# blacksnail789521/IMM-TSF

Measured on AMD Instinct MI355X. Metric: forecast windows/sec (train fwd+bwd) on ragged 64-entity batch, higher is better.
Workload: dtype bf16

## Files before the change

imm-tsf_amd/csrc/capi.hip:

```cpp
#include "../../include/immtsf.h"
#include "attn.hpp"
#include "gemm.hpp"
#include "rowops.hpp"
#include "seam_small.hpp"
#include "tail.hpp"
#include "block_util.hpp"
#include <atomic>

namespace { std::atomic<int> g_side_enabled{0}; }

extern "C" {

int immtsf_side_stream_enabled(void) { return g_side_enabled; }
int immtsf_set_side_stream(int32_t on) { g_side_enabled.store(on ? 1 : 0); return 0; }

int immtsf_gemm(int32_t layout, int32_t precision, const float* A, int32_t lda, const float* B, int32_t ldb, float* C,
                int32_t ldc, const float* bias, int32_t M, int32_t N, int32_t K, float alpha, int32_t accumulate,
                int32_t act, immtsf_stream_t stream) {
    if (!A || !B || !C || layout < 0 || layout > 2) return IMMTSF_EINVAL;
    GemmArgs g = gemm_args(M, N, K, lda, ldb, ldc);
    set_problem(g, 0, A, B, C, bias);
    g.alpha = alpha;
    g.accumulate = accumulate;
    g.act = act;
// ... 126 lines not shown

int immtsf_softmax_rows_backward(float* dA, const float* P, int32_t B, int32_t H, int32_t L, int32_t S, float p_drop,
                                 uint64_t seed, uint64_t site, const uint64_t* seed_step_dev, immtsf_stream_t stream) {
    if (!dA || !P) return IMMTSF_EINVAL;
    DropCfg d = mk_drop(p_drop, seed);
    d.seed_dev = seed_step_dev;
    return launch_softmax_rows_bwd(dA, P, B, H, L, S, d, site, static_cast<hipStream_t>(stream));
}

int immtsf_attention_short_forward(const float* qkv, int32_t B, int32_t L, int32_t H, int32_t E, float scale, int32_t causal,
                                   float p_drop, uint64_t seed, uint64_t site, const uint64_t* seed_step_dev, float* out,
                                   immtsf_stream_t stream) {
    if (!qkv || !out || B < 0 || L <= 0 || H <= 0 || E <= 0) return IMMTSF_EINVAL;
    DropCfg d = mk_drop(p_drop, seed);
    d.seed_dev = seed_step_dev;
    return launch_attn_short_fwd(qkv, B, L, H, E, scale, causal, d, site, out, static_cast<hipStream_t>(stream));
}

int immtsf_attention_short_backward(const float* qkv, const float* dout, int32_t B, int32_t L, int32_t H, int32_t E, float scale,
                                    int32_t causal, float p_drop, uint64_t seed, uint64_t site, const uint64_t* seed_step_dev,
                                    float* dqkv, immtsf_stream_t stream) {
    if (!qkv || !dout || !dqkv || B < 0 || L <= 0 || H <= 0 || E <= 0) return IMMTSF_EINVAL;
    DropCfg d = mk_drop(p_drop, seed);
    d.seed_dev = seed_step_dev;
    return launch_attn_short_bwd(qkv, dout, B, L, H, E, scale, causal, d, site, dqkv, static_cast<hipStream_t>(stream));
}

int immtsf_seam_route(int32_t rows, int32_t d, int32_t PW) { return seam_p_fwd_shape_ok(rows, d, PW) ? 1 : 0; }

int immtsf_seam_p_bf16(const void* A, const void* W, const float* bias, float* P, int32_t rows, int32_t d, int32_t PW, immtsf_stream_t stream) {
    return launch_seam_p_fwd(A, W, bias, P, rows, d, PW, static_cast<hipStream_t>(stream));
}

int immtsf_layernorm_backward_lowrank(const float* G, int32_t ldg, int32_t PW, const float* basis, int32_t rows, int32_t d, const float* gamma,
                                      const float* xhat, const void* xhat_h, const float* rstd, float* dx, void* dxh, float p_drop,
                                      const void* keep, int32_t keep_T, const uint8_t* row_flag, int32_t flag_div, float* dgamma, float* dbeta,
                                      float* dxsum, float* scratch, size_t scratch_bytes, int32_t form, immtsf_stream_t stream) {
    if (scratch_bytes < (size_t)256 * 3 * d * sizeof(float) || (form != 0 && form != 1)) return IMMTSF_EINVAL;
    if (p_drop > 0.f && !keep) return IMMTSF_EINVAL;
    return launch_layernorm_bwd_lr(G, ldg, PW, basis, rows, d, gamma, xhat, xhat_h, rstd, dx, dxh, mk_drop(p_drop, 0), 0, dgamma, dbeta, dxsum,
                                   scratch, row_flag, flag_div, static_cast<hipStream_t>(stream), keep, keep_T, form);
}

int immtsf_layernorm_forward(const float* x, int32_t rows, int32_t d, const float* gamma, const float* beta, float eps,
                             float* xhat, float* rstd, float* z, float p_drop, uint64_t seed, uint64_t site,
                             immtsf_stream_t stream) {
    if (!x || !gamma || !beta || !z || d <= 0) return IMMTSF_EINVAL;
    return launch_layernorm_fwd(x, rows, d, gamma, beta, eps, xhat, rstd, z, mk_drop(p_drop, seed), site,
                                static_cast<hipStream_t>(stream));
}

int immtsf_layernorm_backward(float* dz_dy, int32_t rows, int32_t d, const float* gamma, const float* xhat,
                              const float* rstd, float* dx, float* dgamma, float* dbeta, float* scratch, float p_drop,
                              uint64_t seed, uint64_t site, immtsf_stream_t stream) {
    if (!dz_dy || !gamma || !xhat || !rstd || !dx || d <= 0) return IMMTSF_EINVAL;
    hipStream_t s = static_cast<hipStream_t>(stream);
    CHECK(launch_layernorm_bwd(dz_dy, rows, d, gamma, xhat, rstd, dx, mk_drop(p_drop, seed), site, s));
    if (dgamma && dbeta) {
        if (!scratch) return IMMTSF_EINVAL;
        return launch_colsum2(dz_dy, xhat, rows, d, d, dgamma, dbeta, scratch, s);
    }
    if (dgamma) {
        if (!scratch) return IMMTSF_EINVAL;
        CHECK(launch_colsum(dz_dy, xhat, rows, nullptr, d, d, dgamma, 0, scratch, s));
    }
    if (dbeta) {
// ... 172 lines not shown
```

imm-tsf_amd/csrc/seam_small.hip:

```cpp
#include "seam_small.hpp"

namespace {

template <int NT>
__global__ __launch_bounds__(256) void seam_p_fwd_kernel(const bf16_t* __restrict__ A, const bf16_t* __restrict__ W, const float* __restrict__ bias,
                                                          float* __restrict__ out, int rows, int d, int PW) {
    __shared__ f32x4 red[3][NT][64];
    const int tid = threadIdx.x, lane = tid & 63, wave = tid >> 6, fr = lane & 15, fq = lane >> 4;
    const int row = blockIdx.x * 16 + fr;
    const bool rok = row < rows;
    const bf16_t* ap = A + (size_t)(rok ? row : 0) * d + fq * 8;
    const bf16_t* wp[NT];
    bool wok[NT];
#pragma unroll
    for (int j = 0; j < NT; ++j) {
        wok[j] = j * 16 + fr < PW;
        wp[j] = W + (size_t)(wok[j] ? j * 16 + fr : 0) * d + fq * 8;
    }
    f32x4 acc[NT];
#pragma unroll
    for (int j = 0; j < NT; ++j) acc[j] = f32x4{0.f, 0.f, 0.f, 0.f};
    bf16x8 zero;
#pragma unroll
    for (int e = 0; e < 8; ++e) zero[e] = (bf16_t)0.0f;
    const int nk = d >> 5;
#pragma unroll 4
    for (int ks = wave; ks < nk; ks += 4) {
        const bf16x8 a = rok ? *reinterpret_cast<const bf16x8*>(ap + ks * 32) : zero;
#pragma unroll
        for (int j = 0; j < NT; ++j) {
            const bf16x8 b = wok[j] ? *reinterpret_cast<const bf16x8*>(wp[j] + ks * 32) : zero;
            acc[j] = __builtin_amdgcn_mfma_f32_16x16x32_bf16(a, b, acc[j], 0, 0, 0);
        }
    }
    if (wave > 0) {
#pragma unroll
        for (int j = 0; j < NT; ++j) red[wave - 1][j][lane] = acc[j];
    }
    __syncthreads();
    if (wave > 0) return;
#pragma unroll
    for (int j = 0; j < NT; ++j) {
#pragma unroll
        for (int w = 0; w < 3; ++w) acc[j] += red[w][j][lane];
        const int n = j * 16 + fr;
        if (n >= PW) continue;
        const float b = bias ? bias[n] : 0.f;
#pragma unroll
        for (int r = 0; r < 4; ++r) {
            const int orow = blockIdx.x * 16 + fq * 4 + r;
            if (orow < rows) out[(size_t)orow * PW + n] = acc[j][r] + b;
        }
    }
}

constexpr int SEAM_MIN_ROWS = 512, SEAM_MAX_ROWS = 8192;

}

bool seam_p_fwd_shape_ok(int rows, int d, int PW) {
    return rows >= SEAM_MIN_ROWS && rows < SEAM_MAX_ROWS && PW >= 1 && PW <= 64 && d >= 32 && d <= 1024 && (d & 31) == 0;
}
bool seam_p_fwd_ok(int rows, int d, int PW, const void* A, const void* W, const void* out) {
    const uintptr_t al = reinterpret_cast<uintptr_t>(A) | reinterpret_cast<uintptr_t>(W);
    return seam_p_fwd_shape_ok(rows, d, PW) && (al & 15) == 0 && A && W && out;
}

int launch_seam_p_fwd(const void* A, const void* W, const float* bias, float* out, int rows, int d, int PW, hipStream_t s) {
    if (!seam_p_fwd_ok(rows, d, PW, A, W, out)) return IMMTSF_EUNSUPPORTED;
    const bf16_t* a = static_cast<const bf16_t*>(A);
    const bf16_t* w = static_cast<const bf16_t*>(W);
    const dim3 grid((rows + 15) / 16);
    switch ((PW + 15) / 16) {
        case 1: hipLaunchKernelGGL((seam_p_fwd_kernel<1>), grid, dim3(256), 0, s, a, w, bias, out, rows, d, PW); break;
        case 2: hipLaunchKernelGGL((seam_p_fwd_kernel<2>), grid, dim3(256), 0, s, a, w, bias, out, rows, d, PW); break;
        case 3: hipLaunchKernelGGL((seam_p_fwd_kernel<3>), grid, dim3(256), 0, s, a, w, bias, out, rows, d, PW); break;
        default: hipLaunchKernelGGL((seam_p_fwd_kernel<4>), grid, dim3(256), 0, s, a, w, bias, out, rows, d, PW); break;
    }
    IMMTSF_LAUNCH_CHECK();
    return IMMTSF_OK;
}
```

imm-tsf_amd/csrc/seam_small.hpp:

```cpp
#pragma once
#include "common.hpp"

bool seam_p_fwd_shape_ok(int rows, int d, int PW);
bool seam_p_fwd_ok(int rows, int d, int PW, const void* A, const void* W, const void* out);
int launch_seam_p_fwd(const void* A, const void* W, const float* bias, float* out, int rows, int d, int PW, hipStream_t s);
```

imm-tsf_amd/csrc/xrank.hip:

```cpp
#include "../../include/immtsf.h"
#include "gemm.hpp"
#include "rowops.hpp"
#include "tail.hpp"
#include "block_util.hpp"
#include "t2v_fold.hpp"
#include "eval.hpp"
#include "seam_small.hpp"
#include <math.h>
#include <algorithm>
#include <vector>
#include <type_traits>

namespace {

constexpr int XR = 8;
constexpr int XJ_MAX = 20;
enum { XJ_NN = 0, XJ_NT = 1, XJ_OUTER = 2, XJ_COPY = 3 };
struct XJob {
    int form, nblk;
    const float* L; int lsr, lsn;
    int R;
    const float* W; int ldw, qsn;
    int K, N, M;
    float* out; int osr, osn;
// ... 399 lines not shown
struct XPWs {
    float *AqT, *WHO, *GA, *UA, *Wf, *Wfb;
    unsigned short *Wf16, *E16;
    float *Wc, *bc;
    unsigned short *Wc16, *Wpo16;
    size_t bytes;
};
XPWs carve_xp(const immtsf_fusion_cfg* c, void* base) {
    const XRDims x = xr_dims(c);
    const size_t d = x.d;
    const bool hf = xr_hf(c);
    Carver k(base);
    XPWs w;
    w.AqT = k.take<float>(x.Cq * d);
    w.WHO = k.take<float>(x.C * d);
    w.GA = k.take<float>((size_t)x.H * x.Cq * d);
    w.UA = k.take<float>((size_t)x.H * x.C * d);
    w.Wf = k.take<float>((size_t)x.PW * d);
    w.Wfb = k.take<float>(x.PW);
    w.Wf16 = hf ? k.take<unsigned short>((size_t)x.PW * d) : nullptr;
    w.E16 = hf ? k.take<unsigned short>((size_t)x.B * x.T * d) : nullptr;
    w.Wc = k.take<float>((size_t)x.PW * d);
    w.bc = k.take<float>(x.PW);
    w.Wc16 = hf ? k.take<unsigned short>((size_t)x.PW * d) : nullptr;
    w.Wpo16 = hf ? k.take<unsigned short>(d * d) : nullptr;
    w.bytes = k.bytes();
    return w;
}
struct XPScratch {
    float *dWf, *dWfb, *T1, *RW, *dAqT, *dWHO;
    float *dWc, *dbc;
    unsigned short *dP16, *dWc16;
    void* sk;
    size_t skb, bytes;
};
XPScratch carve_xp_scratch(const immtsf_fusion_cfg* c, void* base) {
    const XRDims x = xr_dims(c);
    const size_t d = x.d, BT = (size_t)x.B * x.T;
    const bool hf = xr_hf(c);
    Carver k(base);
    XPScratch s;
    s.dWf = k.take<float>((size_t)x.PW * d);
    s.dWfb = k.take<float>(x.PW);
    s.T1 = k.take<float>((size_t)x.H * x.Cq * d);
    s.RW = k.take<float>((size_t)x.H * x.C * d);
    s.dAqT = k.take<float>(x.Cq * d);
    s.dWHO = k.take<float>(x.C * d);
    s.dP16 = hf ? k.take<unsigned short>(BT * x.PW) : nullptr;
    s.dWc = k.take<float>((size_t)x.PW * d);
    s.dbc = k.take<float>(x.PW);
    s.dWc16 = hf ? k.take<unsigned short>((size_t)x.PW * d) : nullptr;
    s.skb = hf ? immtsf_gemm3_tn_ws_bytes(x.PW, (int)d, (int)BT) : 0;
    s.sk = s.skb ? k.take<unsigned char>(s.skb) : nullptr;
    s.bytes = k.bytes();
    return s;
}

struct XQDims { int B, T, C, H, PW, Wd, wpb, TB, parts, psh; float kappa; };
struct XQWs {
    float *lse, *xhat, *rstd, *slabs;
    unsigned int* ticket;
    size_t bytes;
};
inline int xq_wpb(const XRDims& x) {
    int wpb = 256 / x.T;
    if (wpb < 1) wpb = 1;
    const size_t per = xq_lds_floats(x) * sizeof(float);
    while (wpb > 1 && per * wpb > XQ_LDS_MAX) --wpb;
    while (wpb > 1 && cdiv(x.B, wpb) < 256) --wpb;
    return wpb;
}
XQWs carve_xq(const immtsf_fusion_cfg* c, void* base) {
    const XRDims x = xr_dims(c);
    const size_t BT = (size_t)x.B * x.T;
    Carver k(base);
    XQWs w;
    w.lse = k.take<float>(BT * x.H);
    w.xhat = k.take<float>(BT * x.C);
    w.rstd = k.take<float>(BT);
    w.slabs = k.take<float>((size_t)cdiv(x.B, xq_wpb(x)) * 3 * x.C);
    w.ticket = k.take<unsigned int>(4);
    w.bytes = k.bytes();
    return w;
}

struct DropL { uint64_t seed; float p, inv_keep; };
// ... 1024 lines not shown

int immtsf_mmf_xrank_p_backward_data_z(const immtsf_fusion_cfg* cfg, const immtsf_xadd_params* p, const float* proj_w, const float* proj_b,
                                       const float* Z, const float* dP, float* dZ, void* workspace, size_t workspace_bytes, void* scratch,
                                       size_t scratch_bytes, immtsf_stream_t stream) {
    if (!xr_supported(cfg) || !p || !proj_w || !proj_b || !Z || !dP || !dZ || !workspace || !scratch) return IMMTSF_EINVAL;
    XPWs w = carve_xp(cfg, workspace);
    XPScratch sc = carve_xp_scratch(cfg, scratch);
    if (workspace_bytes < w.bytes || scratch_bytes < sc.bytes) return IMMTSF_EWORKSPACE;
    hipStream_t s = static_cast<hipStream_t>(stream);
    const XRDims x = xr_dims(cfg);
    const int d = x.d, BT = x.B * x.T, prec = cfg->precision;
    const bool hf = xr_hf(cfg);
    Mat Wpo;
    CHECK(weight_mat(hf, proj_w, (size_t)d * d, w.Wpo16, s, &Wpo));
    Mat dPm = cmat(dP), Zm = cmat(Z, hf ? (cfg->aux_h ? cfg->aux_h : static_cast<const void*>(w.E16)) : nullptr);
    const bool seed_only = cfg->bwd_phase != 0 && !(cfg->bwd_phase & IMMTSF_BWD_PHASE_A);
    if (hf && !cfg->aux_h && !seed_only) CHECK(launch_f32_to_bf16(Z, w.E16, (size_t)BT * d, s));
    if (hf && cfg->in_h) {
        dPm.h = const_cast<void*>(cfg->in_h);
    } else if (hf) {
        if (!seed_only) CHECK(launch_f32_to_bf16(dP, sc.dP16, (size_t)BT * x.PW, s));
        dPm.h = sc.dP16;
    }
    const bool do_data = cfg->bwd_phase == 0 || (cfg->bwd_phase & IMMTSF_BWD_PHASE_A), do_seed = cfg->bwd_phase == 0 || (cfg->bwd_phase & IMMTSF_BWD_WGRAD_A);
    if (do_data && !(cfg->form & IMMTSF_FORM_LOWRANK_OUT)) {
        if (rank_expand_ok(BT, d, x.PW, w.Wc, d, dZ, hf ? cfg->out_h : nullptr)) {
            CHECK(launch_rank_expand(dP, x.PW, w.Wc, d, dZ, hf ? cfg->out_h : nullptr, BT, d, x.PW, s));
        } else {
            GemmArgs g = gemm_args(BT, d, x.PW, x.PW, d, d);
            set_problem2(g, 0, dPm, mat(w.Wc, w.Wc16), mat(dZ, hf ? cfg->out_h : nullptr), nullptr);
            CHECK(immtsf_launch_gemm(GEMM_NN, prec, g, s));
        }
    }
    if (do_seed) {
        GemmArgs g = gemm_args(x.PW, d, BT, x.PW, d, d);
        set_problem2(g, 0, dPm, Zm, mat(sc.dWc), nullptr, sc.dbc);
        g.c_prezeroed = 0;
        g.ws = sc.sk; g.ws_bytes = sc.skb;
        CHECK(immtsf_launch_gemm(GEMM_TN, prec, g, s));
        if (hf) CHECK(launch_f32_to_bf16(sc.dWc, sc.dWc16, (size_t)x.PW * d, s));
    }
    return IMMTSF_OK;
}

int immtsf_mmf_xrank_lowrank_basis(const immtsf_fusion_cfg* cfg, void* workspace, size_t workspace_bytes, const float** basis, int32_t* rank) {
    if (!xr_supported(cfg) || !workspace || !basis || !rank) return IMMTSF_EINVAL;
    XPWs w = carve_xp(cfg, workspace);
    if (workspace_bytes < w.bytes) return IMMTSF_EWORKSPACE;
    *basis = w.Wc;
    *rank = xr_dims(cfg).PW;
    return IMMTSF_OK;
}

int immtsf_mmf_xrank_p_backward_pre_z(const immtsf_fusion_cfg* cfg, const float* proj_w, const float* proj_b, void* workspace,
                                      size_t workspace_bytes, void* scratch, size_t scratch_bytes, float* g_proj_w, float* g_proj_b,
                                      immtsf_stream_t stream) {
    if (!xr_supported(cfg) || !proj_w || !proj_b || !workspace || !scratch || !g_proj_w || !g_proj_b) return IMMTSF_EINVAL;
    XPWs w = carve_xp(cfg, workspace);
    XPScratch sc = carve_xp_scratch(cfg, scratch);
    if (workspace_bytes < w.bytes || scratch_bytes < sc.bytes) return IMMTSF_EWORKSPACE;
    hipStream_t s = static_cast<hipStream_t>(stream);
    const XRDims x = xr_dims(cfg);
    const int d = x.d, prec = cfg->precision;
    const bool hf = xr_hf(cfg);
    Mat Wpo;
    CHECK(weight_mat(hf, proj_w, (size_t)d * d, w.Wpo16, s, &Wpo));
    {
// ... 231 lines not shown
```

imm-tsf_amd/immtsf/_lib.py:

```python
from __future__ import annotations

import ctypes as C
import os

_HERE = os.path.dirname(os.path.abspath(__file__))
LIB_PATH = os.path.join(_HERE, "libimmtsf_hip.so")

ABI_VERSION = 7
AMP_SCRATCH_FLOATS = 2056
FORM_NO_PROJ = 16
FORM_HALF_OUT = 32
FORM_LOWRANK_OUT = 64
BWD_PHASE_A, BWD_PHASE_B, BWD_PHASE_C = 1, 2, 4
BWD_WGRAD_A, BWD_WGRAD_B, BWD_WGRAD_C = 16, 32, 64


class ImmtsfError(RuntimeError):
    pass


_ERR = {-1: "IMMTSF_EINVAL (bad dimension / null pointer)", -2: "IMMTSF_EWORKSPACE (workspace too small)",
        -3: "IMMTSF_EUNSUPPORTED (shape outside kernel limits)"}

c_f32p = C.c_void_p
c_u8p = C.c_void_p
c_i32p = C.c_void_p
c_stream = C.c_void_p


class FusionCfg(C.Structure):
    _fields_ = [("B", C.c_int32), ("N", C.c_int32), ("T", C.c_int32), ("C", C.c_int32), ("d_m", C.c_int32),
                ("d", C.c_int32), ("H", C.c_int32), ("precision", C.c_int32), ("training", C.c_int32),
                ("p_drop", C.c_float), ("kappa", C.c_float), ("seed", C.c_uint64), ("seed_step_dev", C.c_void_p), ("grads_prezeroed", C.c_int32),
                ("form", C.c_int32), ("in_h", C.c_void_p), ("aux_h", C.c_void_p), ("out_h", C.c_void_p), ("sched_flag", C.c_void_p),
                ("bwd_phase", C.c_int32), ("reserved0", C.c_int32), ("note_index", C.c_void_p), ("lr_grad", C.c_void_p)]


class LowRankGrad(C.Structure):
    _fields_ = [("coef", C.c_void_p), ("basis", C.c_void_p), ("rank", C.c_int32), ("ld", C.c_int32)]


def _ptr_struct(name, fields):
    return type(name, (C.Structure,), {"_fields_": [(f, C.c_void_p) for f in fields], "FIELDS": tuple(fields)})


# ... 413 lines not shown
    "immtsf_debug_gemm2_config": (C.c_int, [C.c_int32, C.c_int32, C.c_int32]),
    "immtsf_gemm3_bf16": (C.c_int, [C.c_int32, C.c_void_p, C.c_int32, C.c_void_p, C.c_int32, c_f32p, C.c_int32, C.c_void_p,
                                    C.c_int32, c_f32p, c_f32p, c_i32p, C.c_int32, C.c_int32, C.c_int32, C.c_int32, C.c_float,
                                    C.c_int32, c_i32p, c_stream]),
    "immtsf_debug_gemm3_config": (C.c_int, [C.c_int32, C.c_int32]),
    "immtsf_debug_last_gemm_launch": (C.c_int, [C.c_void_p]),
    "immtsf_gemm3_tn_workspace_bytes": (C.c_size_t, [C.c_int32, C.c_int32, C.c_int32]),
    "immtsf_gemm3_tn_bf16": (C.c_int, [C.c_void_p, C.c_int32, C.c_void_p, C.c_int32, c_f32p, C.c_int32, c_f32p, C.c_int32, C.c_int32,
                                       C.c_int32, C.c_float, C.c_int32, c_i32p, C.c_void_p, C.c_size_t, c_stream]),
    "immtsf_adam_step_dev": (C.c_int, [c_f32p, c_f32p, c_f32p, c_f32p, C.c_uint64, C.c_float, C.c_float, C.c_float,
                                       C.c_float, C.c_float, C.c_void_p, C.c_float, c_f32p, C.c_void_p, c_stream]),
    "immtsf_adam_step_dev_zero": (C.c_int, [c_f32p, c_f32p, c_f32p, c_f32p, C.c_uint64, C.c_float, C.c_float, C.c_float,
                                       C.c_float, C.c_float, C.c_void_p, C.c_float, c_f32p, C.c_void_p, c_stream]),
    "immtsf_adam_step_guarded": (C.c_int, [c_f32p, c_f32p, c_f32p, c_f32p, C.c_uint64, C.c_float, C.c_float, C.c_float,
                                           C.c_float, C.c_float, C.c_void_p, C.c_float, c_f32p, C.c_void_p, C.c_void_p, C.c_int32, c_stream]),
    "immtsf_adam_sqnorm": (C.c_int, [c_f32p, C.c_uint64, c_f32p, C.c_void_p, C.c_void_p, c_stream]),
    "immtsf_adam_apply": (C.c_int, [c_f32p, c_f32p, c_f32p, c_f32p, C.c_uint64, C.c_float, C.c_float, C.c_float, C.c_float, C.c_float,
                                    C.c_int32, C.c_void_p, C.c_float, c_f32p, C.c_void_p, c_stream]),
    "immtsf_adam_step": (C.c_int, [c_f32p, c_f32p, c_f32p, c_f32p, C.c_uint64, C.c_float, C.c_float, C.c_float,
                                   C.c_float, C.c_float, C.c_int32, C.c_float, c_f32p, c_stream]),
    "immtsf_adam_prepare": (C.c_int, [c_f32p, C.c_void_p, C.c_uint64, c_f32p, C.c_void_p, C.c_void_p, C.c_void_p, C.c_void_p, C.c_void_p,
                                      c_f32p, C.c_void_p, c_stream]),
    "immtsf_flag_wait_ge_multi": (C.c_int, [C.c_int32, C.c_void_p, C.c_int32, C.c_void_p, C.c_int32, C.c_void_p, C.c_int32, c_stream]),
    "immtsf_adam_range": (C.c_int, [c_f32p, c_f32p, C.c_void_p, c_f32p, c_f32p, C.c_uint64, C.c_uint64, C.c_uint64, C.c_float, C.c_float,
                                    C.c_float, C.c_float, C.c_float, C.c_void_p, C.c_float, c_f32p, C.c_int32, C.c_void_p, c_stream]),
    "immtsf_adam_prepare_scaled": (C.c_int, [c_f32p, C.c_void_p, C.c_uint64, c_f32p, C.c_void_p, C.c_void_p, C.c_void_p, C.c_void_p,
                                             C.c_void_p, c_f32p, C.c_void_p, c_f32p, c_f32p, c_f32p, C.c_float, c_stream]),
    "immtsf_adam_range_scaled": (C.c_int, [c_f32p, c_f32p, C.c_void_p, c_f32p, c_f32p, C.c_uint64, C.c_uint64, C.c_uint64, C.c_float,
                                           C.c_float, C.c_float, C.c_float, C.c_float, C.c_void_p, c_f32p, C.c_int32, C.c_void_p, c_stream]),
    "immtsf_loss_scale_update": (C.c_int, [c_f32p, C.c_void_p, c_f32p, C.c_float, C.c_float, C.c_int32, c_stream]),
    "immtsf_guard_pack": (C.c_int, [C.c_void_p, C.c_void_p, C.c_int32, c_stream]),
    "immtsf_seam_route": (C.c_int, [C.c_int32] * 3),
    "immtsf_seam_p_bf16": (C.c_int, [C.c_void_p, C.c_void_p, c_f32p, c_f32p, C.c_int32, C.c_int32, C.c_int32, c_stream]),
    "immtsf_layernorm_backward_lowrank": (C.c_int, [c_f32p, C.c_int32, C.c_int32, c_f32p, C.c_int32, C.c_int32, c_f32p, c_f32p, C.c_void_p, c_f32p,
                                                    c_f32p, C.c_void_p, C.c_float, C.c_void_p, C.c_int32, C.c_void_p, C.c_int32, c_f32p, c_f32p,
                                                    c_f32p, c_f32p, C.c_size_t, C.c_int32, c_stream]),
}

def abi_structs():
    return [FusionCfg, T2VParams, RecAvgParams, XAddParams, GRParams, TTCNParams, GCNParams, DecoderParams, Time2VecParams,
            EncoderLayerCfg, EncoderLayerParams, FFNBlockCfg, FFNBlockParams, Store, NoteIndex, LowRankGrad, LatentODEDims, NeuralFlowDims]


_lib = None


def load():
    global _lib
    if _lib is not None:
        return _lib
    global LIB_PATH
    LIB_PATH = os.environ.get("IMMTSF_LIB", LIB_PATH)
    if not os.path.exists(LIB_PATH):
        raise ImmtsfError(
            f"{LIB_PATH} not found: build it with `python -c 'import __graft_entry__ as g; g.build()'` "
            f"or `make -C imm-tsf_amd/csrc`.  There is no CPU fallback.")
    lib = C.CDLL(LIB_PATH)
    for name, (res, args) in _PROTOS.items():
        try:
            fn = getattr(lib, name)
        except AttributeError as e:
            raise ImmtsfError(f"{LIB_PATH} does not export {name}; rebuild it") from e
        fn.restype = res
        fn.argtypes = args
    if lib.immtsf_abi_version() != ABI_VERSION:
        raise ImmtsfError("libimmtsf_hip.so ABI version mismatch; rebuild it")
# ... 28 lines not shown
```

imm-tsf_amd/immtsf/config.py:

```python
import os
import threading

_PRECISIONS = {"fp32": 0, "bf16": 1}

precision = os.environ.get("IMMTSF_PRECISION", "fp32")

nan_check = os.environ.get("IMMTSF_NAN_CHECK", "deferred")


def precision_code(p=None) -> int:
    p = precision if p is None else p
    if p not in _PRECISIONS:
        raise ValueError(f"precision must be one of {sorted(_PRECISIONS)}, got {p!r}")
    return _PRECISIONS[p]


_lock = threading.Lock()
_base_seed = None
_counter = 0


def manual_seed(seed: int):
    global _base_seed, _counter
    with _lock:
# ... 13 lines not shown
        x = (x * 0xBF58476D1CE4E5B9) & 0xFFFFFFFFFFFFFFFF
        x ^= x >> 27
        x = (x * 0x94D049BB133111EB) & 0xFFFFFFFFFFFFFFFF
        x ^= x >> 31
        return x


_device_counters = {}


def enable_device_counters(device):
    import torch
    key = str(device)
    if key not in _device_counters:
        _device_counters[key] = (torch.zeros(1, dtype=torch.int64, device=device),
                                 torch.zeros(1, dtype=torch.int64, device=device))
    return _device_counters[key]


def disable_device_counters(device=None):
    if device is None:
        _device_counters.clear()
    else:
        _device_counters.pop(str(device), None)


def dropout_counter_ptr(device):
    c = _device_counters.get(str(device))
    return None if c is None else c[1].data_ptr()

xattn_rank = True
xattn_fused_loss = True
fuse_tail = "auto"
seam_graph = True
t2v_form = "auto"
note_index = True
gr_split = True
z_handover = os.environ.get("IMMTSF_Z_HANDOVER", "1") != "0"
attn_mid = True
eval_engine = os.environ.get("IMMTSF_EVAL_ENGINE", "0") == "1"
dlinear_fused = os.environ.get("IMMTSF_DLINEAR_FUSED", "1") != "0"
timemixer_fused = os.environ.get("IMMTSF_TIMEMIXER_FUSED", "1") != "0"
ttm_fused = os.environ.get("IMMTSF_TTM_FUSED", "1") != "0"
informer_fused = os.environ.get("IMMTSF_INFORMER_FUSED", "1") != "0"
cru_fused = os.environ.get("IMMTSF_CRU_FUSED", "1") != "0"
timellm_fused = os.environ.get("IMMTSF_TIMELLM_FUSED", "1") != "0"
timellm_bert_fp32 = os.environ.get("IMMTSF_TIMELLM_BERT_FP32", "0") == "1"
frozen_products = os.environ.get("IMMTSF_FROZEN_PRODUCTS", "fp32")
_FROZEN_PRODUCTS = ("fp32", "split")


def frozen_split(precision_code_: int) -> bool:
    if frozen_products not in _FROZEN_PRODUCTS:
        raise ValueError(f"frozen_products must be one of {sorted(_FROZEN_PRODUCTS)}, got {frozen_products!r}")
    return precision_code_ == 0 and frozen_products == "split"
timellm_prompt_fused = os.environ.get("IMMTSF_TIMELLM_PROMPT_FUSED", "1") != "0"
timellm_reprogram_fused = os.environ.get("IMMTSF_TIMELLM_REPROGRAM_FUSED", "1") != "0"
note_embed_fused = os.environ.get("IMMTSF_NOTE_EMBED_FUSED", "1") != "0"
note_embed_fp32_min_notes = int(os.environ.get("IMMTSF_NOTE_EMBED_FP32_MIN_NOTES", "2"))
bert_embed_fp32_min_notes = int(os.environ.get("IMMTSF_BERT_EMBED_FP32_MIN_NOTES", "2"))
llama_embed_fp32_min_notes = int(os.environ.get("IMMTSF_LLAMA_EMBED_FP32_MIN_NOTES", "1"))
latentode_fused = os.environ.get("IMMTSF_LATENTODE_FUSED", "1") != "0"
neuralflow_fused = os.environ.get("IMMTSF_NEURALFLOW_FUSED", "1") != "0"
resident_loader = os.environ.get("IMMTSF_RESIDENT_LOADER", "1") != "0"
optim_amp = os.environ.get("IMMTSF_OPTIM_AMP", "1") != "0"
```

imm-tsf_amd/immtsf/ops.py:

```python
from __future__ import annotations

import ctypes as C

import torch

from . import _lib, config, step_plan
from ._lib import DecoderParams, FusionCfg, GCNParams, GRParams, NoteIndex, RecAvgParams, T2VParams, TTCNParams, XAddParams, check, ptr, stream_ptr


def _need_gpu(*ts):
    for t in ts:
        if t is None:
            continue
        if not t.is_cuda:
            raise _lib.ImmtsfError("immtsf ops need tensors on the GPU (HIP); there is no CPU fallback")
        if t.dtype not in (torch.float32, torch.uint8, torch.bool, torch.int32):
            raise _lib.ImmtsfError(f"unsupported dtype {t.dtype}; the HIP path takes fp32 tensors")


def _c(t):
    return None if t is None else t.contiguous()


def _struct(cls, tensors):
# ... 572 lines not shown
                                                  stream), "mmf_xrank_fold_z")
            else:
                check(lib.immtsf_mmf_xrank_fold(C.byref(cfg), C.byref(ps), ptr(bHO), ptr(ws), ws.numel(), stream), "mmf_xrank_fold")
        folded = 1 if step_plan.current().fold(fold, ws, bHO) else 0
        if proj is not None:
            _need_gpu(*proj)
            check(lib.immtsf_mmf_xrank_p_forward_z(C.byref(cfg), C.byref(ps), ptr(proj[0]), ptr(proj[1]), ptr(E), ptr(P), ptr(bHO), ptr(ws),
                                                   ws.numel(), folded, stream_ptr()), "mmf_xrank_p_forward_z")
        else:
            check(lib.immtsf_mmf_xrank_p_forward(C.byref(cfg), C.byref(ps), ptr(E), ptr(P), ptr(bHO), ptr(ws), ws.numel(),
                                                 folded, stream_ptr()), "mmf_xrank_p_forward")
        ctx.cfg, ctx.ws = cfg, ws
        ctx.sinks = _sinks_of(params)
        ctx.done_hook = done_hook
        ctx.has_proj = proj is not None
        ctx.proj_sinks = _sinks_of(proj) if proj is not None else None
        ctx.save_for_backward(E, *params[:9], *(proj or ()))
        return P, bHO

    @staticmethod
    def backward(ctx, dP, dbHO):
        lib = _lib.load()
        E, *params9 = ctx.saved_tensors
        proj = None
        if ctx.has_proj:
            proj, params9 = params9[9:11], params9[:9]
            pgrads, prets = _grad_buffers(proj, ctx.proj_sinks)
        params = list(params9) + [None, None]
        grads, rets = _grad_buffers(params, ctx.sinks)
        dE = torch.empty_like(E)
        cfg = ctx.cfg
        lowrank = ctx.lowrank and proj is not None and config.z_handover
        cfg.form = (cfg.form | _lib.FORM_LOWRANK_OUT) if lowrank else (cfg.form & ~_lib.FORM_LOWRANK_OUT)
        sc = _bytes(lib.immtsf_mmf_xrank_p_scratch_bytes(C.byref(cfg)), E.device)
        ps, gs = _struct(XAddParams, params), _struct(XAddParams, grads)
        dP = dP.contiguous()
        dbHO = torch.zeros(cfg.C, dtype=torch.float32, device=E.device) if dbHO is None else dbHO.contiguous()
        dE_h = None
        if _bf16_dataflow(cfg.precision, cfg.d):
            dP_h = _reg_take(_shadows, dP)
            cfg.in_h = None if dP_h is None else dP_h.data_ptr()
            cfg.aux_h = None if ctx.E_h is None else ctx.E_h.data_ptr()
            if proj is None:
                dE_h = torch.empty(dE.shape, dtype=torch.bfloat16, device=dE.device)
                cfg.out_h = dE_h.data_ptr()
            else:
                cfg.out_h = None

        ws0 = ctx.ws

        def params_chain(stream, first=0, last=3, keep=(params, grads)):
            if proj is not None and first == 0:
                check(lib.immtsf_mmf_xrank_p_backward_pre_z(C.byref(cfg), ptr(proj[0]), ptr(proj[1]), ptr(ws0), ws0.numel(), ptr(sc), sc.numel(),
                                                            ptr(pgrads[0]), ptr(pgrads[1]), stream), "mmf_xrank_p_backward_pre_z")
            check(lib.immtsf_mmf_xrank_p_backward_params(C.byref(cfg), C.byref(ps), ptr(dbHO), ptr(ws0), ws0.numel(), ptr(sc), sc.numel(),
                                                         C.byref(gs), first, last, stream), "mmf_xrank_p_backward_params")

        def data_half(part=0, stream=None):
            if proj is not None:
                cfg.bwd_phase = part
                check(lib.immtsf_mmf_xrank_p_backward_data_z(C.byref(cfg), C.byref(ps), ptr(proj[0]), ptr(proj[1]), ptr(E), ptr(dP), ptr(dE),
                                                             ptr(ctx.ws), ctx.ws.numel(), ptr(sc), sc.numel(),
                                                             stream_ptr() if stream is None else stream),
                      "mmf_xrank_p_backward_data_z")
                cfg.bwd_phase = 0
            else:
# ... 3292 lines not shown
```

include/immtsf.h:

```cpp
#ifndef IMMTSF_H
#define IMMTSF_H

#include <stddef.h>
#include <stdint.h>

#ifdef __cplusplus
extern "C" {
#endif

#define IMMTSF_ABI_VERSION 7
#define IMMTSF_T2V_FOLD_MIN_ROWS 8192
#define IMMTSF_FORM_NO_PROJ 16
#define IMMTSF_FORM_HALF_OUT 32
#define IMMTSF_FORM_LOWRANK_OUT 64

#define IMMTSF_OK 0
#define IMMTSF_EINVAL (-1)
#define IMMTSF_EWORKSPACE (-2)
#define IMMTSF_EUNSUPPORTED (-3)

typedef void* immtsf_stream_t;

int immtsf_abi_version(void);
int immtsf_instance_norm(const float* x, int32_t B, int32_t L, int32_t C, float* xn, float* means, float* stdev, immtsf_stream_t stream);
int immtsf_notes_stage(const float* emb, int32_t d_m, const int32_t* src_rows, const int32_t* total, int32_t max_rows, void* X_h, int32_t ldx,
                       const float* tau, const int32_t* rowmap, int32_t dt, const float* lin_w, const float* lin_b, const float* per_w,
                       const float* per_b, immtsf_stream_t stream);
#define IMMTSF_ABI_NSTRUCTS 18
int immtsf_abi_sizes(int32_t* out, int32_t max);

typedef struct immtsf_fusion_cfg {
    int32_t B, N, T, C, d_m, d, H;
    int32_t precision;
    int32_t training;
    float p_drop;
    float kappa;
    uint64_t seed;
    const uint64_t* seed_step_dev;
    int32_t grads_prezeroed;
    int32_t form;
    const void* in_h;
    const void* aux_h;
    void* out_h;
    int32_t* sched_flag;
    int32_t bwd_phase;
    int32_t reserved0;
    const struct immtsf_note_index* note_index;
// ... 550 lines not shown
int immtsf_time2vec_forward(const float* t, int32_t rows, int32_t d, const float* w0, const float* b0, const float* w,
                            const float* b, float* out, immtsf_stream_t stream);
int immtsf_time2vec_backward(const float* t, int32_t rows, int32_t d, const float* w, const float* b, const float* dout,
                             float* dw0, float* db0, float* dw, float* db, float* scratch, int32_t accumulate,
                             immtsf_stream_t stream);
int immtsf_bf16_twin_register(const float* base, void* twin, size_t count);
int immtsf_bf16_twin_unregister(const float* base);
int immtsf_bf16_twin_enable(int32_t on);
int immtsf_f32_to_bf16(const float* src, void* dst, size_t n, immtsf_stream_t stream);
int immtsf_bf16_to_f32(const void* src, float* dst, size_t n, immtsf_stream_t stream);
int immtsf_linear_bf16_forward(int32_t nl, const float* x, void* x16, const float* const* W, void* const* w16, const float* const* b,
                               float* const* y, int32_t M, int32_t N, int32_t K, int32_t act, immtsf_stream_t stream);
int immtsf_linear_bf16_backward(int32_t nl, const void* x16, const float* const* W, void* const* w16, const float* const* dy, void* dy16,
                                float* dx, float* const* dW, float* const* db, int32_t M, int32_t N, int32_t K,
                                int32_t grads_prezeroed, immtsf_stream_t stream);
int immtsf_gemm_batched(int32_t layout, int32_t precision, const float* A, int32_t lda, int64_t sA_o, int64_t sA_i,
                        const float* B, int32_t ldb, int64_t sB_o, int64_t sB_i, float* C, int32_t ldc, int64_t sC_o,
                        int64_t sC_i, int32_t n_outer, int32_t n_inner, int32_t M, int32_t N, int32_t K, float alpha,
                        immtsf_stream_t stream);
int immtsf_softmax_rows_forward(float* sc, float* A, int32_t B, int32_t H, int32_t L, int32_t S, const uint8_t* live,
                                float p_drop, uint64_t seed, uint64_t site, int32_t causal, const uint64_t* seed_step_dev,
                                immtsf_stream_t stream);
int immtsf_softmax_rows_backward(float* dA, const float* P, int32_t B, int32_t H, int32_t L, int32_t S, float p_drop,
                                 uint64_t seed, uint64_t site, const uint64_t* seed_step_dev, immtsf_stream_t stream);
#define IMMTSF_ATTN_SHORT_MAX 8
int immtsf_attention_short_forward(const float* qkv, int32_t B, int32_t L, int32_t H, int32_t E, float scale, int32_t causal,
                                   float p_drop, uint64_t seed, uint64_t site, const uint64_t* seed_step_dev, float* out,
                                   immtsf_stream_t stream);
int immtsf_attention_short_backward(const float* qkv, const float* dout, int32_t B, int32_t L, int32_t H, int32_t E, float scale,
                                    int32_t causal, float p_drop, uint64_t seed, uint64_t site, const uint64_t* seed_step_dev,
                                    float* dqkv, immtsf_stream_t stream);
int immtsf_seam_route(int32_t rows, int32_t d, int32_t PW);
int immtsf_seam_p_bf16(const void* A, const void* W, const float* bias, float* P, int32_t rows, int32_t d, int32_t PW, immtsf_stream_t stream);
int immtsf_layernorm_backward_lowrank(const float* G, int32_t ldg, int32_t PW, const float* basis, int32_t rows, int32_t d, const float* gamma,
                                      const float* xhat, const void* xhat_h, const float* rstd, float* dx, void* dxh, float p_drop,
                                      const void* keep, int32_t keep_T, const uint8_t* row_flag, int32_t flag_div, float* dgamma, float* dbeta,
                                      float* dxsum, float* scratch, size_t scratch_bytes, int32_t form, immtsf_stream_t stream);
int immtsf_layernorm_forward(const float* x, int32_t rows, int32_t d, const float* gamma, const float* beta, float eps,
                             float* xhat, float* rstd, float* z, float p_drop, uint64_t seed, uint64_t site,
                             immtsf_stream_t stream);
int immtsf_layernorm_backward(float* dz_dy, int32_t rows, int32_t d, const float* gamma, const float* xhat,
                              const float* rstd, float* dx, float* dgamma, float* dbeta, float* scratch,
                              float p_drop, uint64_t seed, uint64_t site, immtsf_stream_t stream);
int immtsf_dropout_mask(uint64_t seed, uint64_t site, uint64_t n, float p_drop, uint8_t* out, immtsf_stream_t stream);
#define IMMTSF_SITE_T2V_ATTN 1
#define IMMTSF_SITE_T2V_OUT 2
#define IMMTSF_SITE_REC_OUT 3
#define IMMTSF_SITE_XADD_ATTN 4
#define IMMTSF_SITE_XADD_OUT 5
#define IMMTSF_SITE_GR_OUT 6
#define IMMTSF_SITE_LAYER_BASE 16

int immtsf_adam_step(float* param, const float* grad, float* exp_avg, float* exp_avg_sq, uint64_t n, float lr,
                     float beta1, float beta2, float eps, float weight_decay, int32_t step, float max_norm,
                     float* norm_scratch, immtsf_stream_t stream);
int immtsf_adam_step_dev(float* param, const float* grad, float* exp_avg, float* exp_avg_sq, uint64_t n, float lr,
                         float beta1, float beta2, float eps, float weight_decay, int64_t* step_dev, float max_norm,
                         float* norm_scratch, uint64_t* dropout_step_dev, immtsf_stream_t stream);

int immtsf_adam_step_dev_zero(float* param, float* grad, float* exp_avg, float* exp_avg_sq, uint64_t n, float lr, float beta1,
                              float beta2, float eps, float weight_decay, int64_t* step_dev, float max_norm, float* norm_scratch,
                              uint64_t* dropout_step_dev, immtsf_stream_t stream);

int immtsf_adam_step_guarded(float* param, float* grad, float* exp_avg, float* exp_avg_sq, uint64_t n, float lr, float beta1,
                             float beta2, float eps, float weight_decay, int64_t* step_dev, float max_norm, float* norm_scratch,
                             uint64_t* dropout_step_dev, const int32_t* skip_flag, int32_t zero_grad, immtsf_stream_t stream);
// ... 167 lines not shown
```

Before: 156,900.

## Add split-K bf16 MFMA kernel for seam weight-gradient with slab reduction

Adds a dedicated kernel for the small-PW weight-gradient product dWc = dP^T Z (plus the bias gradient via an MFMA against a ones vector). Rows are split into 128-row slabs written to workspace, and a second kernel sums them and emits fp32 and bf16 outputs. The xrank backward path uses it by default when shapes fit, falling back to the generic GEMM otherwise. The aim is to replace a poorly occupied tall-skinny GEMM with a parallel split-K scheme. In exchange it needs extra workspace, an extra launch and a slab reduction pass.

New measurement: 157,900 (median of 4 runs). No clear change (+0.6%).

```diff
diff --git a/imm-tsf_amd/csrc/capi.hip b/imm-tsf_amd/csrc/capi.hip
--- a/imm-tsf_amd/csrc/capi.hip
+++ b/imm-tsf_amd/csrc/capi.hip
@@ -182,6 +182,13 @@
     return launch_seam_p_fwd(A, W, bias, P, rows, d, PW, static_cast<hipStream_t>(stream));
 }
 
+int immtsf_seam_wc_route(int32_t rows, int32_t d, int32_t PW) { return seam_wc_bwd_shape_ok(rows, d, PW) ? 1 : 0; }
+size_t immtsf_seam_wc_ws_bytes(int32_t rows, int32_t d, int32_t PW) { return seam_wc_bwd_ws_bytes(rows, d, PW); }
+int immtsf_seam_wc_bf16(const void* dP, const void* Z, float* dWc, void* dWc_h, float* dbc, int32_t rows, int32_t d, int32_t PW, void* ws,
+                        size_t ws_bytes, immtsf_stream_t stream) {
+    return launch_seam_wc_bwd(dP, Z, dWc, dWc_h, dbc, rows, d, PW, ws, ws_bytes, static_cast<hipStream_t>(stream));
+}
+
 int immtsf_layernorm_backward_lowrank(const float* G, int32_t ldg, int32_t PW, const float* basis, int32_t rows, int32_t d, const float* gamma,
                                       const float* xhat, const void* xhat_h, const float* rstd, float* dx, void* dxh, float p_drop,
                                       const void* keep, int32_t keep_T, const uint8_t* row_flag, int32_t flag_div, float* dgamma, float* dbeta,
diff --git a/imm-tsf_amd/csrc/seam_small.hip b/imm-tsf_amd/csrc/seam_small.hip
--- a/imm-tsf_amd/csrc/seam_small.hip
+++ b/imm-tsf_amd/csrc/seam_small.hip
@@ -56,6 +56,105 @@
 
 constexpr int SEAM_MIN_ROWS = 512, SEAM_MAX_ROWS = 8192;
 
+constexpr int WC_ROWS = 128, WC_COLS = 64, WC_ZP = WC_COLS / 2 + 2;
+typedef unsigned short u16x8 __attribute__((ext_vector_type(8)));
+
+template <int MT>
+__global__ __launch_bounds__(256) void seam_wc_bwd_kernel(const bf16_t* __restrict__ dP, const bf16_t* __restrict__ Z, float* __restrict__ slabs,
+                                                           float* __restrict__ bslabs, int rows, int d, int PW) {
+    constexpr int PP = MT * 8 + 2;
+    __shared__ __attribute__((aligned(16))) unsigned int Zs[WC_ROWS * WC_ZP];
+    __shared__ __attribute__((aligned(16))) unsigned int Ps[WC_ROWS * PP];
+    const int tid = threadIdx.x, lane = tid & 63, wave = tid >> 6, fr = lane & 15, fq = lane >> 4;
+    const int n0 = blockIdx.x * WC_COLS, r0 = blockIdx.y * WC_ROWS;
+    const uint4 zero4 = make_uint4(0u, 0u, 0u, 0u);
+    constexpr int ZCH = WC_COLS / 8, ZL = WC_ROWS * ZCH / 256, PL = (WC_ROWS * MT * 2 + 255) / 256;
+    uint4 zr[ZL], pr[PL];
+#pragma unroll
+    for (int i = 0; i < ZL; ++i) {
+        const int c = tid + i * 256, row = c / ZCH, col = n0 + (c % ZCH) * 8;
+        zr[i] = (r0 + row < rows && col < d) ? *reinterpret_cast<const uint4*>(Z + (size_t)(r0 + row) * d + col) : zero4;
+    }
+    const int pch = PW >> 3;
+#pragma unroll
+    for (int i = 0; i < PL; ++i) {
+        const int c = tid + i * 256, row = c / (MT * 2), ch = c % (MT * 2);
+        pr[i] = (row < WC_ROWS && r0 + row < rows && ch < pch) ? *reinterpret_cast<const uint4*>(dP + (size_t)(r0 + row) * PW + ch * 8) : zero4;
+    }
+#pragma unroll
+    for (int i = 0; i < ZL; ++i) {
+        const int c = tid + i * 256;
+        uint2* dst = reinterpret_cast<uint2*>(Zs + (c / ZCH) * WC_ZP + (c % ZCH) * 4);
+        dst[0] = make_uint2(zr[i].x, zr[i].y);
+        dst[1] = make_uint2(zr[i].z, zr[i].w);
+    }
+#pragma unroll
+    for (int i = 0; i < PL; ++i) {
+        const int c = tid + i * 256, row = c / (MT * 2), ch = c % (MT * 2);
+        if (row < WC_ROWS) {
+            uint2* dst = reinterpret_cast<uint2*>(Ps + row * PP + ch * 4);
+            dst[0] = make_uint2(pr[i].x, pr[i].y);
+            dst[1] = make_uint2(pr[i].z, pr[i].w);
+        }
+    }
+    __syncthreads();
+    const int nt = n0 + wave * 16;
+    if (nt >= d) return;
+    const unsigned short* Zh = reinterpret_cast<const unsigned short*>(Zs) + wave * 16 + fr;
+    const unsigned short* Ph = reinterpret_cast<const unsigned short*>(Ps) + fr;
+    const bool bsum = blockIdx.x == 0 && wave == 0;
+    bf16x8 ones;
+#pragma unroll
+    for (int e = 0; e < 8; ++e) ones[e] = (bf16_t)1.0f;
+    f32x4 acc[MT], accb[MT];
+#pragma unroll
+    for (int i = 0; i < MT; ++i) acc[i] = accb[i] = f32x4{0.f, 0.f, 0.f, 0.f};
+#pragma unroll
+    for (int ks = 0; ks < WC_ROWS / 32; ++ks) {
+        const int k = ks * 32 + fq * 8;
+        u16x8 bz;
+#pragma unroll
+        for (int e = 0; e < 8; ++e) bz[e] = Zh[(k + e) * (WC_ZP * 2)];
+        const bf16x8 b = __builtin_bit_cast(bf16x8, bz);
+#pragma unroll
+        for (int i = 0; i < MT; ++i) {
+            u16x8 ap;
+#pragma unroll
+            for (int e = 0; e < 8; ++e) ap[e] = Ph[(k + e) * (PP * 2) + i * 16];
+            const bf16x8 a = __builtin_bit_cast(bf16x8, ap);
+            acc[i] = __builtin_amdgcn_mfma_f32_16x16x32_bf16(a, b, acc[i], 0, 0, 0);
+            if (bsum) accb[i] = __builtin_amdgcn_mfma_f32_16x16x32_bf16(a, ones, accb[i], 0, 0, 0);
+        }
+    }
+    float* slab = slabs + (size_t)blockIdx.y * PW * d;
+#pragma unroll
+    for (int i = 0; i < MT; ++i)
+#pragma unroll
+        for (int r = 0; r < 4; ++r) {
+            const int m = i * 16 + fq * 4 + r;
+            if (m >= PW) continue;
+            slab[(size_t)m * d + nt + fr] = acc[i][r];
+            if (bsum && fr == 0) bslabs[(size_t)blockIdx.y * PW + m] = accb[i][r];
+        }
+}
+
+__global__ __launch_bounds__(256) void seam_wc_sum_kernel(const float* __restrict__ slabs, const float* __restrict__ bslabs, int nslab, int n,
+                                                           int PW, float* __restrict__ out, bf16_t* __restrict__ outh, float* __restrict__ bout) {
+    const int i = blockIdx.x * 256 + threadIdx.x;
+    if (i < n) {
+        float a = 0.f;
+#pragma unroll 8
+        for (int s = 0; s < nslab; ++s) a += slabs[(size_t)s * n + i];
+        out[i] = a;
+        if (outh) outh[i] = (bf16_t)a;
+    } else if (i < n + PW) {
+        const int m = i - n;
+        float a = 0.f;
+        for (int s = 0; s < nslab; ++s) a += bslabs[(size_t)s * PW + m];
+        bout[m] = a;
+    }
+}
+
 }
 
 bool seam_p_fwd_shape_ok(int rows, int d, int PW) {
@@ -80,3 +179,34 @@
     IMMTSF_LAUNCH_CHECK();
     return IMMTSF_OK;
 }
+
+bool seam_wc_bwd_shape_ok(int rows, int d, int PW) {
+    return rows >= SEAM_MIN_ROWS && rows < SEAM_MAX_ROWS && PW >= 8 && PW <= 64 && (PW & 7) == 0 && d >= 16 && d <= 1024 && (d & 15) == 0;
+}
+size_t seam_wc_bwd_ws_bytes(int rows, int d, int PW) {
+    if (!seam_wc_bwd_shape_ok(rows, d, PW)) return 0;
+    return (size_t)((rows + WC_ROWS - 1) / WC_ROWS) * ((size_t)PW * d + PW) * sizeof(float);
+}
+
+int launch_seam_wc_bwd(const void* dP, const void* Z, float* dWc, void* dWc16, float* dbc, int rows, int d, int PW, void* ws, size_t ws_bytes,
+                       hipStream_t s) {
+    const uintptr_t al = reinterpret_cast<uintptr_t>(dP) | reinterpret_cast<uintptr_t>(Z) | reinterpret_cast<uintptr_t>(ws);
+    if (!seam_wc_bwd_shape_ok(rows, d, PW) || !dP || !Z || !dWc || !dbc || !ws || (al & 15) != 0) return IMMTSF_EUNSUPPORTED;
+    if (ws_bytes < seam_wc_bwd_ws_bytes(rows, d, PW)) return IMMTSF_EWORKSPACE;
+    const int nslab = (rows + WC_ROWS - 1) / WC_ROWS, n = PW * d;
+    float* slabs = static_cast<float*>(ws);
+    float* bslabs = slabs + (size_t)nslab * n;
+    const bf16_t* p = static_cast<const bf16_t*>(dP);
+    const bf16_t* z = static_cast<const bf16_t*>(Z);
+    const dim3 grid((d + WC_COLS - 1) / WC_COLS, nslab);
+    switch ((PW + 15) / 16) {
+        case 1: hipLaunchKernelGGL((seam_wc_bwd_kernel<1>), grid, dim3(256), 0, s, p, z, slabs, bslabs, rows, d, PW); break;
+        case 2: hipLaunchKernelGGL((seam_wc_bwd_kernel<2>), grid, dim3(256), 0, s, p, z, slabs, bslabs, rows, d, PW); break;
+        case 3: hipLaunchKernelGGL((seam_wc_bwd_kernel<3>), grid, dim3(256), 0, s, p, z, slabs, bslabs, rows, d, PW); break;
+        default: hipLaunchKernelGGL((seam_wc_bwd_kernel<4>), grid, dim3(256), 0, s, p, z, slabs, bslabs, rows, d, PW); break;
+    }
+    IMMTSF_LAUNCH_CHECK();
+    hipLaunchKernelGGL(seam_wc_sum_kernel, dim3((n + PW + 255) / 256), dim3(256), 0, s, slabs, bslabs, nslab, n, PW, dWc, static_cast<bf16_t*>(dWc16), dbc);
+    IMMTSF_LAUNCH_CHECK();
+    return IMMTSF_OK;
+}
diff --git a/imm-tsf_amd/csrc/seam_small.hpp b/imm-tsf_amd/csrc/seam_small.hpp
--- a/imm-tsf_amd/csrc/seam_small.hpp
+++ b/imm-tsf_amd/csrc/seam_small.hpp
@@ -4,3 +4,8 @@
 bool seam_p_fwd_shape_ok(int rows, int d, int PW);
 bool seam_p_fwd_ok(int rows, int d, int PW, const void* A, const void* W, const void* out);
 int launch_seam_p_fwd(const void* A, const void* W, const float* bias, float* out, int rows, int d, int PW, hipStream_t s);
+
+bool seam_wc_bwd_shape_ok(int rows, int d, int PW);
+size_t seam_wc_bwd_ws_bytes(int rows, int d, int PW);
+int launch_seam_wc_bwd(const void* dP, const void* Z, float* dWc, void* dWc16, float* dbc, int rows, int d, int PW, void* ws, size_t ws_bytes,
+                       hipStream_t s);
diff --git a/imm-tsf_amd/csrc/xrank.hip b/imm-tsf_amd/csrc/xrank.hip
--- a/imm-tsf_amd/csrc/xrank.hip
+++ b/imm-tsf_amd/csrc/xrank.hip
@@ -455,7 +455,8 @@
     float *dWc, *dbc;
     unsigned short *dP16, *dWc16;
     void* sk;
-    size_t skb, bytes;
+    void* wcs;
+    size_t skb, wcsb, bytes;
 };
 XPScratch carve_xp_scratch(const immtsf_fusion_cfg* c, void* base) {
     const XRDims x = xr_dims(c);
@@ -475,6 +476,8 @@
     s.dWc16 = hf ? k.take<unsigned short>((size_t)x.PW * d) : nullptr;
     s.skb = hf ? immtsf_gemm3_tn_ws_bytes(x.PW, (int)d, (int)BT) : 0;
     s.sk = s.skb ? k.take<unsigned char>(s.skb) : nullptr;
+    s.wcsb = hf ? seam_wc_bwd_ws_bytes((int)BT, (int)d, x.PW) : 0;
+    s.wcs = s.wcsb ? k.take<float>(s.wcsb / sizeof(float)) : nullptr;
     s.bytes = k.bytes();
     return s;
 }
@@ -1565,7 +1568,9 @@
             CHECK(immtsf_launch_gemm(GEMM_NN, prec, g, s));
         }
     }
-    if (do_seed) {
+    if (do_seed && hf && !(cfg->form & IMMTSF_FORM_SEED_GEMM) && sc.wcsb &&
+        launch_seam_wc_bwd(dPm.h, Zm.h, sc.dWc, sc.dWc16, sc.dbc, BT, d, x.PW, sc.wcs, sc.wcsb, s) == IMMTSF_OK) {
+    } else if (do_seed) {
         GemmArgs g = gemm_args(x.PW, d, BT, x.PW, d, d);
         set_problem2(g, 0, dPm, Zm, mat(sc.dWc), nullptr, sc.dbc);
         g.c_prezeroed = 0;
diff --git a/imm-tsf_amd/immtsf/_lib.py b/imm-tsf_amd/immtsf/_lib.py
--- a/imm-tsf_amd/immtsf/_lib.py
+++ b/imm-tsf_amd/immtsf/_lib.py
@@ -11,6 +11,7 @@
 FORM_NO_PROJ = 16
 FORM_HALF_OUT = 32
 FORM_LOWRANK_OUT = 64
+FORM_SEED_GEMM = 128
 BWD_PHASE_A, BWD_PHASE_B, BWD_PHASE_C = 1, 2, 4
 BWD_WGRAD_A, BWD_WGRAD_B, BWD_WGRAD_C = 16, 32, 64
 
@@ -490,6 +491,10 @@
     "immtsf_guard_pack": (C.c_int, [C.c_void_p, C.c_void_p, C.c_int32, c_stream]),
     "immtsf_seam_route": (C.c_int, [C.c_int32] * 3),
     "immtsf_seam_p_bf16": (C.c_int, [C.c_void_p, C.c_void_p, c_f32p, c_f32p, C.c_int32, C.c_int32, C.c_int32, c_stream]),
+    "immtsf_seam_wc_route": (C.c_int, [C.c_int32] * 3),
+    "immtsf_seam_wc_ws_bytes": (C.c_size_t, [C.c_int32] * 3),
+    "immtsf_seam_wc_bf16": (C.c_int, [C.c_void_p, C.c_void_p, c_f32p, C.c_void_p, c_f32p, C.c_int32, C.c_int32, C.c_int32, C.c_void_p, C.c_size_t,
+                            c_stream]),
     "immtsf_layernorm_backward_lowrank": (C.c_int, [c_f32p, C.c_int32, C.c_int32, c_f32p, C.c_int32, C.c_int32, c_f32p, c_f32p, C.c_void_p, c_f32p,
                                                     c_f32p, C.c_void_p, C.c_float, C.c_void_p, C.c_int32, C.c_void_p, C.c_int32, c_f32p, c_f32p,
                                                     c_f32p, c_f32p, C.c_size_t, C.c_int32, c_stream]),
diff --git a/imm-tsf_amd/immtsf/config.py b/imm-tsf_amd/immtsf/config.py
--- a/imm-tsf_amd/immtsf/config.py
+++ b/imm-tsf_amd/immtsf/config.py
@@ -69,6 +69,7 @@
 xattn_rank = True
 xattn_fused_loss = True
 fuse_tail = "auto"
+seam_wc = os.environ.get("IMMTSF_SEAM_WC", "1") != "0"
 seam_graph = True
 t2v_form = "auto"
 note_index = True
diff --git a/imm-tsf_amd/immtsf/ops.py b/imm-tsf_amd/immtsf/ops.py
--- a/imm-tsf_amd/immtsf/ops.py
+++ b/imm-tsf_amd/immtsf/ops.py
@@ -628,6 +628,7 @@
         cfg = ctx.cfg
         lowrank = ctx.lowrank and proj is not None and config.z_handover
         cfg.form = (cfg.form | _lib.FORM_LOWRANK_OUT) if lowrank else (cfg.form & ~_lib.FORM_LOWRANK_OUT)
+        cfg.form = (cfg.form & ~_lib.FORM_SEED_GEMM) if config.seam_wc else (cfg.form | _lib.FORM_SEED_GEMM)
         sc = _bytes(lib.immtsf_mmf_xrank_p_scratch_bytes(C.byref(cfg)), E.device)
         ps, gs = _struct(XAddParams, params), _struct(XAddParams, grads)
         dP = dP.contiguous()
diff --git a/include/immtsf.h b/include/immtsf.h
--- a/include/immtsf.h
+++ b/include/immtsf.h
@@ -13,6 +13,7 @@
 #define IMMTSF_FORM_NO_PROJ 16
 #define IMMTSF_FORM_HALF_OUT 32
 #define IMMTSF_FORM_LOWRANK_OUT 64
+#define IMMTSF_FORM_SEED_GEMM 128
 
 #define IMMTSF_OK 0
 #define IMMTSF_EINVAL (-1)
@@ -629,6 +630,10 @@
                                     float* dqkv, immtsf_stream_t stream);
 int immtsf_seam_route(int32_t rows, int32_t d, int32_t PW);
 int immtsf_seam_p_bf16(const void* A, const void* W, const float* bias, float* P, int32_t rows, int32_t d, int32_t PW, immtsf_stream_t stream);
+int immtsf_seam_wc_route(int32_t rows, int32_t d, int32_t PW);
+size_t immtsf_seam_wc_ws_bytes(int32_t rows, int32_t d, int32_t PW);
+int immtsf_seam_wc_bf16(const void* dP, const void* Z, float* dWc, void* dWc_h, float* dbc, int32_t rows, int32_t d, int32_t PW, void* ws,
+                        size_t ws_bytes, immtsf_stream_t stream);
 int immtsf_layernorm_backward_lowrank(const float* G, int32_t ldg, int32_t PW, const float* basis, int32_t rows, int32_t d, const float* gamma,
                                       const float* xhat, const void* xhat_h, const float* rstd, float* dx, void* dxh, float p_drop,
                                       const void* keep, int32_t keep_T, const uint8_t* row_flag, int32_t flag_div, float* dgamma, float* dbeta,
```
